# falgon/jpezy

Measured on AMD Instinct MI355X. Metric: Mpixels/s encode (FDCT+quant), higher is better.
Workload: dtype f32+f64 guard; 1 GPU; BASELINE configs[1]: single 4096x4096 random-pixel frame encode; width=4096, height=4096, mode=color, ring_batches=6, inputs=iid uniform u8 r,g,b planes resident in HBM, parallelism=frames x1, submission=one launch per step, the K steps captured once and replayed as a hipGraph

## Files before the change

jpezy_amd/csrc/jpezy_entropy.hip:

```cpp
#include <hip/hip_runtime.h>
#include <stdint.h>

#include "jpezy_entropy.h"
#include "../../include/jpezy_constants.h"

namespace jpezy_dev {
namespace entropy {

struct alignas(16) LdsTables {
    uint32_t dc[2][16];
    uint32_t ac[2][256];
    uint32_t fast[2][1024];
};
static_assert(sizeof(LdsTables) <= sizeof(CodeTables) && sizeof(LdsTables) % 16 == 0, "table images must match");

__device__ __forceinline__ void load_tables(LdsTables& L, const CodeTables* T)
{
    const uint4* src = reinterpret_cast<const uint4*>(T);
    uint4* dst = reinterpret_cast<uint4*>(&L);
    for (unsigned i = threadIdx.x; i < sizeof(LdsTables) / 16; i += blockDim.x) dst[i] = src[i];
}

__device__ __forceinline__ uint32_t wg256_exclusive_scan(uint32_t v, uint32_t* total)
{
    __shared__ uint32_t wsum[4];
    const int lane = threadIdx.x & 63, wv = threadIdx.x >> 6;
    uint32_t inc = v;
#pragma unroll
    for (int d = 1; d < 64; d <<= 1) {
        const uint32_t o = __shfl_up(inc, d, 64);
        if (lane >= d) inc += o;
    }
    if (lane == 63) wsum[wv] = inc;
    __syncthreads();
    uint32_t woff = 0, tot = 0;
#pragma unroll
    for (int k = 0; k < 4; ++k) {
        if (k < wv) woff += wsum[k];
        tot += wsum[k];
    }
    *total = tot;
    return woff + inc - v;
}

template <class W>
__device__ __forceinline__ void code_ac(uint32_t m, int base, const int16_t* z, int& prev, const uint32_t* ac, const uint32_t* fast,
                                        uint32_t zrl, W& w, unsigned& amax)
{
    int lz = __builtin_clz(m | 1u);
    int vnext = z[base + lz];
#pragma unroll 1
    while (m) {
        const int n = base + lz, v = vnext;
        m &= 0x7FFFFFFFu >> lz;
        lz = __builtin_clz(m | 1u);
        vnext = z[base + lz];
        w.read_up_to(n);
        int run = n - prev - 1;
        prev = n;
        const unsigned v32 = (unsigned)(v + 32);
        uint32_t e = fast[((unsigned)run << 6) + v32];
        const bool slow = v32 > 63u || run > 15;
        if (slow) {
            const unsigned a = (unsigned)(v < 0 ? -v : v);
            amax = a > amax ? a : amax;
            int sz = 32 - __builtin_clz(a);
            sz = sz > 10 ? 10 : sz;
            if (run > 15) {
                for (int r = run >> 4; r > 0; --r) w.put(zrl >> 8, (int)(zrl & 0xFF));
                run &= 15;
            }
            const uint32_t g = ac[(run << 4) | sz];
            e = ((((g >> 8) << sz) | ((uint32_t)(v + (v >> 31)) & ((1u << sz) - 1u))) << 5) | ((g & 0xFF) + (uint32_t)sz);
        }
        w.put(e >> 5, (int)(e & 31u));
    }
}

template <class W>
__device__ __forceinline__ bool code_block(const int16_t* z, int pred, const uint32_t* dc, const uint32_t* ac, const uint32_t* fast, W& w)
{
    unsigned amax = 0;
    bool ok = true;
    uint32_t mhi = 0, mlo = 0;
    int dcv = 0;
    if (z) {
#pragma unroll
        for (int k = 0; k < 8; ++k) {
            const uint4 c = reinterpret_cast<const uint4*>(z)[k];
            const uint32_t wd[4] = { c.x, c.y, c.z, c.w };
            uint32_t m8 = 0;
#pragma unroll
            for (int j = 0; j < 4; ++j) {
                m8 |= ((wd[j] & 0xFFFFu) ? 1u : 0u) << (7 - 2 * j);
                m8 |= ((wd[j] >> 16) ? 1u : 0u) << (6 - 2 * j);
            }
            if (k < 4) mhi |= m8 << (24 - 8 * k); else mlo |= m8 << (24 - 8 * (k - 4));
            if (k == 0) dcv = (int)(short)(c.x & 0xFFFFu);
        }
        mhi &= 0x7FFFFFFFu;
    }
    {
        const int diff = dcv - pred;
        const unsigned a = (unsigned)(diff < 0 ? -diff : diff);
        int di = a ? 32 - __builtin_clz(a) : 0;
        ok = di <= 11;
        di = di > 11 ? 11 : di;
        const uint32_t e = dc[di];
        w.put(((e >> 8) << di) | ((uint32_t)(diff + (diff >> 31)) & ((1u << di) - 1u)), (int)(e & 0xFF) + di);
    }
    int prev = 0;
    if (z) {
        const uint32_t zrl = ac[0xF0];
        code_ac(mhi, 0, z, prev, ac, fast, zrl, w, amax);
        code_ac(mlo, 32, z, prev, ac, fast, zrl, w, amax);
    }
    w.read_up_to(63);
    if (prev != 63) {
        const uint32_t e = ac[0x00];
        w.put(e >> 8, (int)(e & 0xFF));
    }
    return ok && amax <= 1023u;
}

constexpr int CHUNK = 64;

__device__ __forceinline__ unsigned count_ff(uint32_t x)
{
    const uint32_t z = ~x;
    uint32_t y = (z & 0x7F7F7F7Fu) + 0x7F7F7F7Fu;
    y = ~(y | z | 0x7F7F7F7Fu);
    return (unsigned)__builtin_popcount(y);
}

constexpr int WG = 256;
constexpr int ROW = 144, ROW_DATA = 16, ROW_LAST_WORD = 34;
constexpr unsigned TILE_STREAM_WORDS = 256 * kMaxBlockBytes / 4;

struct RowWriter {
    unsigned long long acc;
    int nacc, wj2, npos;
    unsigned long long bad;
    char* row12;
    __device__ __forceinline__ void init(uint32_t* r)
    {
        row12 = reinterpret_cast<char*>(r) + 12; acc = 0; nacc = 0; bad = 0;
        wj2 = -6; npos = 0;
    }
    __device__ __forceinline__ void read_up_to(int n) { npos = n; }
    __device__ __forceinline__ void word(uint32_t v, bool due)
    {
        const unsigned long long dm = __builtin_amdgcn_ballot_w64(due), lm = __builtin_amdgcn_ballot_w64(wj2 <= npos);
        if (due && wj2 <= npos) *reinterpret_cast<uint32_t*>(row12 + 2 * wj2) = v;
        bad |= dm & ~lm;
        wj2 += due ? 2 : 0;
    }
    __device__ __forceinline__ void put(uint32_t bits, int n)
    {
        acc = (acc << n) | bits;
        const int t = nacc + n;
        nacc = t & 31;
        word((uint32_t)(acc >> nacc), t >= 32);
    }
    __device__ __forceinline__ unsigned bits() const { return 16u * (unsigned)(wj2 + 6) + (unsigned)nacc; }
    __device__ __forceinline__ void finish()
    {
        word((uint32_t)(acc << (32 - nacc)), nacc > 0);
    }
    __device__ __forceinline__ bool overflowed() const { return (bad >> (threadIdx.x & 63u)) & 1ull; }
};

struct DirectWriter {
    unsigned long long acc;
    int nacc;
    unsigned w;
    uint32_t* S;
    bool skip;
    __device__ __forceinline__ void init(uint32_t* tile_stream, unsigned bitoff)
    {
        S = tile_stream; w = bitoff >> 5; nacc = (int)(bitoff & 31u); acc = 0; skip = nacc != 0;
    }
    __device__ __forceinline__ void read_up_to(int) {}
    __device__ __forceinline__ void put(uint32_t bits, int n)
    {
        acc = (acc << n) | bits;
        nacc += n;
        if (nacc >= 32) {
            nacc -= 32;
            if (!skip) S[w] = (uint32_t)(acc >> nacc);
            skip = false;
            ++w;
        }
    }
};

template <bool RST, unsigned CODED = 6u, unsigned LUMA = 4u>
__global__ __launch_bounds__(WG) void code_tiles_kernel(Job job, uint32_t* S, uint32_t* tile_total, unsigned* status)
{
    __shared__ LdsTables L;
    __shared__ __attribute__((aligned(16))) char tile[WG * ROW];
    const unsigned tid = threadIdx.x, frame = blockIdx.y;
    load_tables(L, job.tables + (size_t)frame * job.tables_stride);
    const unsigned nblk = job.blocks_per_frame;
    unsigned g0, nb;
    bool interval_start = false;
    if constexpr (RST) {
        const unsigned bpi = job.restart * CODED, tpi = restart_tpi<CODED>(job.restart), iv = blockIdx.x / tpi, j = blockIdx.x - iv * tpi;
        const unsigned i0 = iv * bpi, ilen = nblk - i0 < bpi ? nblk - i0 : bpi;
        g0 = i0 + j * (unsigned)WG;
        nb = ilen - j * (unsigned)WG < (unsigned)WG ? ilen - j * (unsigned)WG : (unsigned)WG;
        interval_start = j == 0;
    } else {
        g0 = blockIdx.x * (unsigned)WG;
        nb = nblk - g0 < (unsigned)WG ? nblk - g0 : (unsigned)WG;
    }
    const int16_t* fc = job.coeffs + (size_t)frame * job.coeffs_per_frame;
    const bool valid = tid < nb;
    int pred = 0, table = 0;
    const int16_t* zg = nullptr;
    if (valid) {
        const unsigned g = g0 + tid, mcu = g / CODED, i = g - mcu * CODED;
        table = i < LUMA ? 0 : 1;
        if (!(CODED == 6u && i >= 4 && job.bpm == 4)) {
            zg = fc + ((size_t)mcu * job.bpm + i) * 64;
            if (i >= 1 && i < LUMA) pred = zg[-64];
            else if (RST ? !(interval_start && tid < CODED) : mcu != 0) pred = i == 0 ? zg[-(job.bpm - (int)(LUMA - 1u)) * 64] : zg[-job.bpm * 64];
        }
    }
    if (CODED != 6u || job.bpm == 6) {
        const uint4* src = reinterpret_cast<const uint4*>(fc + (size_t)g0 * 64);
        for (unsigned c = tid; c < nb * 8u; c += WG)
            *reinterpret_cast<uint4*>(tile + (c >> 3) * ROW + ROW_DATA + (c & 7u) * 16u) = src[c];
    } else {
        const unsigned g1 = g0 + nb - 1, m0 = g0 / 6u, i0 = g0 - m0 * 6u, m1 = g1 / 6u, i1 = g1 - m1 * 6u;
        const unsigned s0 = i0 < 4 ? m0 * 4u + i0 : (m0 + 1) * 4u, s1 = i1 < 4 ? m1 * 4u + i1 : m1 * 4u + 3u;
        const unsigned nchunks = (s1 + 1 - s0) * 8u;
        const uint4* src = reinterpret_cast<const uint4*>(fc + (size_t)s0 * 64);
        for (unsigned c = tid; c < nchunks; c += WG) {
            const unsigned sb = s0 + (c >> 3), r = (sb >> 2) * 6u + (sb & 3u) - g0;
            *reinterpret_cast<uint4*>(tile + r * ROW + ROW_DATA + (c & 7u) * 16u) = src[c];
        }
    }
    __syncthreads();

    uint32_t* const row = reinterpret_cast<uint32_t*>(tile + tid * ROW);
    unsigned n = 0;
    bool ovf = false;
    if (valid) {
        RowWriter w;
        w.init(row);
        const bool ok = code_block(zg ? reinterpret_cast<const int16_t*>(tile + tid * ROW + ROW_DATA) : nullptr, pred, L.dc[table], L.ac[table],
                                   L.fast[table], w);
        n = w.bits();
        w.finish();
        ovf = w.overflowed();
        if (!ok) atomicOr(status + frame, 1u);
    }
    row[ROW_LAST_WORD + 1] = n;
    uint32_t total;
    const uint32_t o = wg256_exclusive_scan(n, &total);
    const size_t t_index = (size_t)frame * gridDim.x + blockIdx.x;
    if (tid == 0) tile_total[t_index] = total;
    if (!valid) return;

    uint32_t* const Sg = RST ? S + (size_t)frame * ((size_t)((nblk + 255u) / 256u) * TILE_STREAM_WORDS) + (size_t)g0 * (TILE_STREAM_WORDS / 256u)
                             : S + t_index * TILE_STREAM_WORDS;
    const unsigned sh = o & 31u, w0 = o >> 5, end = o + n;
    uint32_t tail = 0;
    unsigned tail_word = 0, tail_fill = 0;
    if (!ovf) {
        const unsigned nwp = (n + 31u) >> 5;
        unsigned k = sh ? 1u : 0u;
        uint32_t prev = sh ? row[0] : 0u;
        for (; ((w0 + k + 1u) << 5) <= end; ++k) {
            const uint32_t cur = k < nwp ? row[k] : 0u;
            Sg[w0 + k] = __builtin_amdgcn_alignbit(prev, cur, sh);
            prev = cur;
        }
        if (((w0 + k) << 5) < end) {
            const uint32_t cur = k < nwp ? row[k] : 0u;
            tail_word = w0 + k;
            tail_fill = end - (tail_word << 5);
            tail = __builtin_amdgcn_alignbit(prev, cur, sh) & ~(0xFFFFFFFFu >> tail_fill);
        }
    } else {
        DirectWriter w;
        w.init(Sg, o);
        (void)code_block(zg, pred, L.dc[table], L.ac[table], L.fast[table], w);
        if (w.nacc > 0 && !w.skip) {
            tail_word = w.w;
            tail_fill = (unsigned)w.nacc;
            tail = (uint32_t)(w.acc << (32 - w.nacc));
        }
    }
    if (tail_fill) {
        unsigned fill = tail_fill;
        for (unsigned j = tid + 1; fill < 32u && j < nb; ++j) {
            const uint32_t* rj = reinterpret_cast<const uint32_t*>(tile + j * ROW);
            tail |= rj[0] >> fill;
            fill += rj[ROW_LAST_WORD + 1];
        }
        Sg[tail_word] = tail;
    }
}

constexpr unsigned ASM_BITS = 256u * (unsigned)CHUNK * 8u;
__global__ __launch_bounds__(256) void tile_bases_kernel(const uint32_t* tile_total, unsigned tpf, unsigned long long* base,
                                                        unsigned long long* bytes, uint32_t* first_tile, unsigned ft_stride,
                                                        unsigned* status, unsigned* latched)
{
    const unsigned f = blockIdx.x, tid = threadIdx.x;
    const uint32_t* tt = tile_total + (size_t)f * tpf;
    unsigned long long* B = base + (size_t)f * (tpf + 1);
    uint32_t* ft = first_tile + (size_t)f * ft_stride;
    unsigned long long carry = 0;
    for (unsigned b0 = 0; b0 < tpf; b0 += 2048u) {
        uint32_t v[8], s = 0;
#pragma unroll
        for (int k = 0; k < 8; ++k) {
            const unsigned t = b0 + tid * 8u + k;
            v[k] = t < tpf ? tt[t] : 0u;
            s += v[k];
        }
        uint32_t total;
        unsigned long long run = carry + wg256_exclusive_scan(s, &total);
#pragma unroll
        for (int k = 0; k < 8; ++k) {
            const unsigned t = b0 + tid * 8u + k;
            if (t < tpf) {
                B[t] = run;
                for (unsigned long long w = (run + ASM_BITS - 1) / ASM_BITS; w * ASM_BITS < run + v[k] && w < ft_stride; ++w) ft[w] = t;
            }
            run += v[k];
        }
        carry += total;
        __syncthreads();
    }
    if (tid == 0) {
        B[tpf] = carry;
        bytes[f] = (carry + 7) >> 3;
        if (latched) {
            latched[f] = status[f];
            status[f] = 0;
        }
    }
}

constexpr unsigned MIN_TILE_BITS = 42u * 32u + 20u;
constexpr int ASM_WIN = 128;
static_assert((unsigned)(ASM_WIN - 2) * MIN_TILE_BITS >= ASM_BITS, "assemble window too small for flat content");
constexpr unsigned MIN_TILE_BITS_444 = 85u * 14u + 4u;
static_assert((unsigned)(ASM_WIN - 2) * MIN_TILE_BITS_444 >= ASM_BITS, "assemble window too small for flat 4:4:4 content");
constexpr unsigned MIN_TILE_BITS_ANY = 256u * 2u;
constexpr int ASM_WIN_ANY = 264;
static_assert((unsigned)(ASM_WIN_ANY - 2) * MIN_TILE_BITS_ANY >= ASM_BITS, "assemble window too small for one-bit codes");
constexpr unsigned ASM_SELF_TILES = 2048;

__device__ __forceinline__ unsigned assemble_chunk(unsigned long long p, unsigned long long bA, unsigned long long eA, const uint32_t* srcA,
                                                   unsigned LB, const uint32_t* srcB, unsigned long long T, uint4* dst)
{
    const unsigned long long qA = p - bA;
    const unsigned LA = (unsigned)(eA - bA), aA = (unsigned)(qA >> 5), sA = (unsigned)(qA & 31u);
    uint32_t wa[17];
#pragma unroll
    for (int k = 0; k < 17; ++k) wa[k] = qA < LA && ((aA + k) << 5) < LA ? srcA[aA + k] : 0u;
    const bool two = LB != 0 && p + CHUNK * 8 > eA;
    const unsigned dB = two ? (unsigned)(eA - p) : 0u, kb = dB >> 5, rb = dB & 31u;
    uint32_t wn[16];
#pragma unroll
    for (int k = 0; k < 16; ++k) wn[k] = two && (unsigned)k >= kb && (((unsigned)k - kb) << 5) < LB ? srcB[(unsigned)k - kb] : 0u;
    uint32_t out[16];
#pragma unroll
    for (int k = 0; k < 16; ++k) {
        uint32_t v = sA ? __builtin_amdgcn_alignbit(wa[k], wa[k + 1], 32u - sA) : wa[k];
        v |= __builtin_amdgcn_alignbit(k > 0 ? wn[k - 1] : 0u, wn[k], rb);
        out[k] = v;
    }
#if JPEZY_PAD_BIT
    {
        const unsigned pad = (unsigned)((8 - (T & 7)) & 7);
        if (pad && T > p && T < p + CHUNK * 8) {
            const unsigned kk = (unsigned)((T - p) >> 5), keep = (unsigned)((T - p) & 31u);
#pragma unroll
            for (int k = 0; k < 16; ++k)
                if ((unsigned)k == kk) out[k] |= ((1u << pad) - 1u) << (32u - keep - pad);
        }
    }
#else
    (void)T;
#endif
    unsigned n_ff = 0;
#pragma unroll
    for (int k = 0; k < 16; ++k) n_ff += count_ff(out[k]);
#pragma unroll
    for (int k = 0; k < 4; ++k)
        dst[k] = make_uint4(__builtin_bswap32(out[4 * k]), __builtin_bswap32(out[4 * k + 1]), __builtin_bswap32(out[4 * k + 2]),
                            __builtin_bswap32(out[4 * k + 3]));
    return n_ff;
}

template <bool SELF, int WIN = ASM_WIN>
__global__ __launch_bounds__(256) void assemble_kernel(const uint32_t* S, const uint32_t* tile_total, const unsigned long long* base,
                                                      unsigned long long* bytes, const uint32_t* first_tile, unsigned tpf,
                                                      unsigned ft_stride, uint32_t* U, size_t u_stride_words, uint32_t* loc,
                                                      uint32_t* ff_tile_total, unsigned* status, unsigned* latched)
{
    __shared__ unsigned long long wb[SELF ? 1 : WIN + 2];
    __shared__ uint32_t pre[SELF ? ASM_SELF_TILES + 2 : 1];
    const unsigned frame = blockIdx.y, tid = threadIdx.x;
    const size_t chunks_per_frame = u_stride_words * 4 / CHUNK, pieces = chunks_per_frame / 256;
    unsigned long long T, nbytes;
    if constexpr (SELF) {
        const uint32_t* tt = tile_total + (size_t)frame * tpf;
        uint32_t v[8], sum = 0;
#pragma unroll
        for (int k = 0; k < 8; ++k) {
            const unsigned t = tid * 8u + k;
            v[k] = t < tpf ? tt[t] : 0u;
            sum += v[k];
        }
        uint32_t total;
        uint32_t run = wg256_exclusive_scan(sum, &total);
#pragma unroll
        for (int k = 0; k < 8; ++k) {
            pre[tid * 8u + k] = run;
            run += v[k];
        }
        if (tid == 255) { pre[ASM_SELF_TILES] = total; pre[ASM_SELF_TILES + 1] = total; }
        __syncthreads();
        T = total;
        nbytes = (T + 7) >> 3;
        if (blockIdx.x == 0 && tid == 0) {
            bytes[frame] = nbytes;
            if (latched) {
                latched[frame] = status[frame];
                status[frame] = 0;
            }
        }
    } else {
        nbytes = bytes[frame];
        T = 0;
#if JPEZY_PAD_BIT
        T = base[(size_t)frame * (tpf + 1) + tpf];
#endif
    }
    for (size_t x = blockIdx.x; x < pieces; x += gridDim.x) {
        const unsigned long long c0 = (unsigned long long)x * 256u, c = c0 + tid;
        if (x != 0 && c0 * CHUNK > nbytes) break;
        unsigned n_ff = 0;
        const unsigned long long p = c * (CHUNK * 8ull);
        uint4* dst = reinterpret_cast<uint4*>(U + (size_t)frame * u_stride_words) + c * (CHUNK / 16);
        if constexpr (SELF) {
            if (c * CHUNK < nbytes) {
                unsigned lo = 0, hi = tpf;
                while (hi - lo > 1) {
                    const unsigned mid = (lo + hi) >> 1;
                    if (pre[mid] <= p) lo = mid; else hi = mid;
                }
                const unsigned t = lo;
                const uint32_t* srcA = S + ((size_t)frame * tpf + t) * TILE_STREAM_WORDS;
                const unsigned LB = t + 1 < tpf ? pre[t + 2] - pre[t + 1] : 0u;
                n_ff = assemble_chunk(p, pre[t], pre[t + 1], srcA, LB, srcA + TILE_STREAM_WORDS, T, dst);
            }
        } else {
            const unsigned t0 = first_tile[(size_t)frame * ft_stride + x];
            const unsigned long long* B = base + (size_t)frame * (tpf + 1);
            __syncthreads();
            for (unsigned i = tid; i < (unsigned)WIN + 2u; i += 256u) wb[i] = B[t0 + i < tpf ? t0 + i : tpf];
            __syncthreads();
            if (c * CHUNK < nbytes) {
                int lo = 0, hi = WIN;
                while (hi - lo > 1) {
                    const int mid = (lo + hi) >> 1;
                    if (wb[mid] <= p) lo = mid; else hi = mid;
                }
                const int t = lo;
                const unsigned tA = t0 + (unsigned)t < tpf ? t0 + (unsigned)t : tpf - 1;
                const uint32_t* srcA = S + ((size_t)frame * tpf + tA) * TILE_STREAM_WORDS;
                const unsigned LB = tA + 1 < tpf ? (unsigned)(wb[t + 2] - wb[t + 1]) : 0u;
                n_ff = assemble_chunk(p, wb[t], wb[t + 1], srcA, LB, srcA + TILE_STREAM_WORDS, T, dst);
            }
        }
        uint32_t total;
        const uint32_t off = wg256_exclusive_scan(n_ff, &total);
        loc[(size_t)frame * chunks_per_frame + c] = off;
        if (tid == 0) ff_tile_total[(size_t)frame * pieces + x] = total;
        __syncthreads();
    }
}

__global__ __launch_bounds__(256) void restart_bases_kernel(const uint32_t* tile_total, unsigned tpf, unsigned tpi, unsigned ni,
                                                           unsigned long long* base, unsigned long long* padsum, unsigned long long* bytes,
                                                           uint32_t* first_tile, unsigned ft_stride, unsigned* status, unsigned* latched)
{
    const unsigned f = blockIdx.x, tid = threadIdx.x;
    const uint32_t* tt = tile_total + (size_t)f * tpf;
    unsigned long long* B = base + (size_t)f * (tpf + 1);
    unsigned long long* P = padsum + (size_t)f * ni;
    uint32_t* ft = first_tile + (size_t)f * ft_stride;
    unsigned long long carry = 0;
    for (unsigned b0 = 0; b0 < tpf; b0 += 2048u) {
        uint32_t v[8], s = 0;
#pragma unroll
        for (int k = 0; k < 8; ++k) {
            const unsigned t = b0 + tid * 8u + k;
            v[k] = t < tpf ? tt[t] : 0u;
            s += v[k];
        }
        uint32_t total;
        unsigned long long run = carry + wg256_exclusive_scan(s, &total);
#pragma unroll
        for (int k = 0; k < 8; ++k) {
            const unsigned t = b0 + tid * 8u + k;
            if (t < tpf) B[t] = run;
            run += v[k];
        }
        carry += total;
        __syncthreads();
    }
    if (tid == 0) B[tpf] = carry;
    __syncthreads();
    carry = 0;
    for (unsigned k0 = 0; k0 < ni; k0 += 2048u) {
        uint32_t v[8], s = 0;
#pragma unroll
        for (int e = 0; e < 8; ++e) {
            const unsigned k = k0 + tid * 8u + e;
            v[e] = k + 1 < ni ? (uint32_t)((0ull - (B[(size_t)(k + 1) * tpi] - B[(size_t)k * tpi])) & 7ull) : 0u;
            s += v[e];
        }
        uint32_t total;
        unsigned long long run = carry + wg256_exclusive_scan(s, &total);
#pragma unroll
        for (int e = 0; e < 8; ++e) {
            const unsigned k = k0 + tid * 8u + e;
            if (k < ni) P[k] = run;
            run += v[e];
        }
        carry += total;
        __syncthreads();
    }
    for (unsigned t = tid; t <= tpf; t += 256u) {
        const unsigned k = t / tpi;
        B[t] += P[k < ni ? k : ni - 1];
    }
    __syncthreads();
    for (unsigned t = tid; t < tpf; t += 256u) {
        const unsigned long long b = B[t], e = B[t + 1];
        for (unsigned long long w = (b + ASM_BITS - 1) / ASM_BITS; w * ASM_BITS < e && w < ft_stride; ++w) ft[w] = t;
    }
    if (tid == 0) {
        bytes[f] = (B[tpf] + 7) >> 3;
        if (latched) {
            latched[f] = status[f];
            status[f] = 0;
        }
    }
}

template <unsigned CODED>
__device__ __forceinline__ unsigned assemble_chunk_restart(unsigned long long p, const unsigned long long* B, const uint32_t* tt, unsigned t,
                                                           unsigned tpf, unsigned tpi, unsigned restart, const uint32_t* Sf,
                                                           unsigned long long T, uint4* dst, unsigned long long& marks, unsigned& k7)
{
    uint32_t out[16];
#pragma unroll
    for (int k = 0; k < 16; ++k) out[k] = 0u;
    marks = 0;
    k7 = 0;
    unsigned long long b = B[t];
    for (unsigned u = t; u < tpf && b < p + CHUNK * 8; ++u) {
        const unsigned long long e = B[u + 1];
        const uint32_t* src = Sf + (size_t)restart_tile_first<CODED>(u, restart) * (TILE_STREAM_WORDS / 256u);
        const unsigned L = tt[u];
        if (u == t) {
            const unsigned long long q = p - b;
            const unsigned a = (unsigned)(q >> 5), sa = (unsigned)(q & 31u);
            uint32_t wa[17];
#pragma unroll
            for (int k = 0; k < 17; ++k) wa[k] = ((a + k) << 5) < L ? src[a + k] : 0u;
#pragma unroll
            for (int k = 0; k < 16; ++k) out[k] = sa ? __builtin_amdgcn_alignbit(wa[k], wa[k + 1], 32u - sa) : wa[k];
        } else {
            const unsigned d = (unsigned)(b - p), kb = d >> 5, rb = d & 31u;
            uint32_t wn[16];
#pragma unroll
            for (int k = 0; k < 16; ++k) wn[k] = (unsigned)k >= kb && (((unsigned)k - kb) << 5) < L ? src[(unsigned)k - kb] : 0u;
#pragma unroll
            for (int k = 0; k < 16; ++k) out[k] |= __builtin_amdgcn_alignbit(k > 0 ? wn[k - 1] : 0u, wn[k], rb);
        }
        const bool ends = (u + 1) % tpi == 0 && u + 1 < tpf;
        if (ends && e <= p + CHUNK * 8) {
            if (!marks) k7 = (u / tpi) & 7u;
            marks |= 1ull << (unsigned)(((e - p) >> 3) - 1);
        }
#if JPEZY_PAD_BIT
        if (ends) {
            const unsigned long long raw = b + L;
            const unsigned pad = (unsigned)(e - raw);
            if (pad && raw < p + CHUNK * 8) {
                const unsigned kk = (unsigned)((raw - p) >> 5), keep = (unsigned)((raw - p) & 31u);
#pragma unroll
                for (int k = 0; k < 16; ++k)
                    if ((unsigned)k == kk) out[k] |= ((1u << pad) - 1u) << (32u - keep - pad);
            }
        }
#endif
        b = e;
    }
#if JPEZY_PAD_BIT
    {
        const unsigned pad = (unsigned)((8 - (T & 7)) & 7);
        if (pad && T > p && T < p + CHUNK * 8) {
            const unsigned kk = (unsigned)((T - p) >> 5), keep = (unsigned)((T - p) & 31u);
#pragma unroll
            for (int k = 0; k < 16; ++k)
                if ((unsigned)k == kk) out[k] |= ((1u << pad) - 1u) << (32u - keep - pad);
        }
    }
#else
    (void)T;
#endif
    unsigned n_ff = 0;
#pragma unroll
    for (int k = 0; k < 16; ++k) n_ff += count_ff(out[k]);
#pragma unroll
    for (int k = 0; k < 4; ++k)
        dst[k] = make_uint4(__builtin_bswap32(out[4 * k]), __builtin_bswap32(out[4 * k + 1]), __builtin_bswap32(out[4 * k + 2]),
                            __builtin_bswap32(out[4 * k + 3]));
    return n_ff + 2u * (unsigned)__builtin_popcountll(marks);
}

template <unsigned CODED>
__global__ __launch_bounds__(256) void assemble_restart_kernel(const uint32_t* S, size_t s_frame_words, const uint32_t* tile_total,
                                                              const unsigned long long* base, const unsigned long long* bytes,
                                                              const uint32_t* first_tile, unsigned tpf, unsigned restart, unsigned ft_stride,
                                                              uint32_t* U, size_t u_stride_words, uint32_t* loc, uint32_t* ff_tile_total,
                                                              unsigned long long* markers)
{
    const unsigned frame = blockIdx.y, tid = threadIdx.x;
    const size_t chunks_per_frame = u_stride_words * 4 / CHUNK, pieces = chunks_per_frame / 256;
    const unsigned long long* B = base + (size_t)frame * (tpf + 1);
    const uint32_t* ft = first_tile + (size_t)frame * ft_stride;
    const unsigned long long nbytes = bytes[frame], T = B[tpf];
    const unsigned tpi = restart_tpi<CODED>(restart);
    for (size_t x = blockIdx.x; x < pieces; x += gridDim.x) {
        const unsigned long long c0 = (unsigned long long)x * 256u, c = c0 + tid;
        if (x != 0 && c0 * CHUNK > nbytes) break;
        unsigned extra = 0, k7 = 0;
        unsigned long long marks = 0;
        const unsigned long long p = c * (CHUNK * 8ull);
        if (c * CHUNK < nbytes) {
            unsigned lo = ft[x], hi = (unsigned long long)(x + 1) * ASM_BITS < T ? ft[x + 1] + 1u : tpf;
            while (hi - lo > 1) {
                const unsigned mid = (lo + hi) >> 1;
                if (B[mid] <= p) lo = mid; else hi = mid;
            }
            uint4* dst = reinterpret_cast<uint4*>(U + (size_t)frame * u_stride_words) + c * (CHUNK / 16);
            extra = assemble_chunk_restart<CODED>(p, B, tile_total + (size_t)frame * tpf, lo, tpf, tpi, restart, S + (size_t)frame * s_frame_words, T,
                                           dst, marks, k7);
        }
        uint32_t total;
        const uint32_t off = wg256_exclusive_scan(extra, &total);
        loc[(size_t)frame * chunks_per_frame + c] = off | (k7 << 29);
        markers[(size_t)frame * chunks_per_frame + c] = marks;
        if (tid == 0) ff_tile_total[(size_t)frame * pieces + x] = total;
        __syncthreads();
    }
}

constexpr int SCAN_T = 256, SCAN_E = 8, SCAN_N = SCAN_T * SCAN_E;

template <typename TIn>
__global__ __launch_bounds__(SCAN_T) void scan_local_kernel(const TIn* in, unsigned long long* out, unsigned long long* totals,
                                                           size_t n)
{
    __shared__ unsigned long long wsum[SCAN_T / 64];
    const size_t base = (size_t)blockIdx.x * SCAN_N + (size_t)threadIdx.x * SCAN_E;
    unsigned long long v[SCAN_E], s = 0;
#pragma unroll
    for (int k = 0; k < SCAN_E; ++k) {
        v[k] = base + k < n ? (unsigned long long)in[base + k] : 0ull;
        s += v[k];
    }
    unsigned long long inc = s;
    const int lane = threadIdx.x & 63, wv = threadIdx.x >> 6;
#pragma unroll
    for (int d = 1; d < 64; d <<= 1) {
        const unsigned long long o = __shfl_up(inc, d, 64);
        if (lane >= d) inc += o;
    }
    if (lane == 63) wsum[wv] = inc;
    __syncthreads();
    unsigned long long woff = 0;
    for (int k = 0; k < wv; ++k) woff += wsum[k];
    unsigned long long run = woff + inc - s;
#pragma unroll
    for (int k = 0; k < SCAN_E; ++k) {
        if (base + k < n) out[base + k] = run;
        run += v[k];
    }
    if (threadIdx.x == SCAN_T - 1) {
        totals[blockIdx.x] = run;
        if (gridDim.x == 1) out[n] = run;
    }
}

__global__ __launch_bounds__(SCAN_T) void scan_add_kernel(unsigned long long* out, const unsigned long long* offs, size_t n,
                                                         unsigned long long* total_slot)
{
    const size_t base = (size_t)blockIdx.x * SCAN_N + (size_t)threadIdx.x * SCAN_E;
    const unsigned long long o = offs[blockIdx.x];
#pragma unroll
    for (int k = 0; k < SCAN_E; ++k)
        if (base + k < n) out[base + k] += o;
    (void)total_slot;
}

size_t scan_tmp_elems(size_t n)
{
    size_t t = 0;
    while (n > 1) {
        n = (n + SCAN_N - 1) / SCAN_N;
        t += n + 1 + n;
        if (n == 1) break;
    }
    return t + 4;
}

__global__ __launch_bounds__(SCAN_T) void scan_finish_kernel(unsigned long long* out, const unsigned long long* totals, size_t n, size_t nb)
{
    __shared__ unsigned long long wsum[SCAN_T / 64];
    unsigned long long sum = 0;
    for (size_t k = threadIdx.x; k < (size_t)blockIdx.x; k += SCAN_T) sum += totals[k];
#pragma unroll
    for (int d = 32; d >= 1; d >>= 1) sum += __shfl_xor(sum, d, 64);
    if ((threadIdx.x & 63) == 0) wsum[threadIdx.x >> 6] = sum;
    __syncthreads();
    unsigned long long o = 0;
#pragma unroll
    for (int k = 0; k < SCAN_T / 64; ++k) o += wsum[k];
    const size_t base = (size_t)blockIdx.x * SCAN_N + (size_t)threadIdx.x * SCAN_E;
#pragma unroll
    for (int k = 0; k < SCAN_E; ++k)
        if (base + k < n) out[base + k] += o;
    if (blockIdx.x == nb - 1 && threadIdx.x == 0) out[n] = o + totals[nb - 1];
}

constexpr size_t SCAN_ONE_WG_MAX = 16 * SCAN_N;
template <typename TIn>
__global__ __launch_bounds__(SCAN_T) void scan_one_wg_kernel(const TIn* in, unsigned long long* out, size_t n)
{
    __shared__ unsigned long long wsum[SCAN_T / 64];
    const int lane = threadIdx.x & 63, wv = threadIdx.x >> 6;
    unsigned long long carry = 0;
    for (size_t b0 = 0; b0 < n; b0 += SCAN_N) {
        const size_t base = b0 + (size_t)threadIdx.x * SCAN_E;
        unsigned long long v[SCAN_E], s = 0;
#pragma unroll
        for (int k = 0; k < SCAN_E; ++k) {
            v[k] = base + k < n ? (unsigned long long)in[base + k] : 0ull;
            s += v[k];
        }
        unsigned long long inc = s;
#pragma unroll
        for (int d = 1; d < 64; d <<= 1) {
            const unsigned long long o = __shfl_up(inc, d, 64);
            if (lane >= d) inc += o;
        }
        if (lane == 63) wsum[wv] = inc;
        __syncthreads();
        unsigned long long woff = 0, tot = 0;
#pragma unroll
        for (int k = 0; k < SCAN_T / 64; ++k) {
            if (k < wv) woff += wsum[k];
            tot += wsum[k];
        }
        unsigned long long run = carry + woff + inc - s;
#pragma unroll
        for (int k = 0; k < SCAN_E; ++k) {
            if (base + k < n) out[base + k] = run;
            run += v[k];
        }
        carry += tot;
        __syncthreads();
    }
    if (threadIdx.x == 0) out[n] = carry;
}

constexpr size_t SCAN_FINISH_MAX_WGS = 4096;

template <typename TIn>
static hipError_t scan_exclusive(const TIn* in, unsigned long long* out, size_t n, unsigned long long* tmp, hipStream_t s)
{
    if (n == 0) return hipMemsetAsync(out, 0, sizeof(unsigned long long), s);
    if (n <= SCAN_ONE_WG_MAX) {
        hipLaunchKernelGGL((scan_one_wg_kernel<TIn>), dim3(1), dim3(SCAN_T), 0, s, in, out, n);
        return hipGetLastError();
    }
    const size_t nb = (n + SCAN_N - 1) / SCAN_N;
    unsigned long long* raw = tmp;
    unsigned long long* scanned = tmp + nb;
    hipLaunchKernelGGL((scan_local_kernel<TIn>), dim3((unsigned)nb), dim3(SCAN_T), 0, s, in, out, raw, n);
    if (nb == 1) return hipGetLastError();
    if (nb <= SCAN_FINISH_MAX_WGS) {
        hipLaunchKernelGGL(scan_finish_kernel, dim3((unsigned)nb), dim3(SCAN_T), 0, s, out, raw, n, nb);
        return hipGetLastError();
    }
    hipError_t e = scan_exclusive<unsigned long long>(raw, scanned, nb, scanned + nb + 1, s);
    if (e != hipSuccess) return e;
    hipLaunchKernelGGL(scan_add_kernel, dim3((unsigned)nb), dim3(SCAN_T), 0, s, out, scanned, n, (unsigned long long*)nullptr);
    return hipMemcpyAsync(out + n, scanned + nb, sizeof(unsigned long long), hipMemcpyDeviceToDevice, s);
}


constexpr int STUFF_WG = 256;
template <bool RST>
__global__ __launch_bounds__(STUFF_WG) void stuff_kernel(const uint32_t* U, size_t u_stride_words, const unsigned long long* frame_bytes,
                                                        const uint32_t* ff_loc, const uint32_t* ff_tile_total, uint8_t* out, size_t out_stride,
                                                        FilePlan plan)
{
    __shared__ uint32_t buf[STUFF_WG * CHUNK * (RST ? 3 : 2) / 4 + 4];
    __shared__ unsigned long long red[2][STUFF_WG / 64];
    uint8_t* const lb = reinterpret_cast<uint8_t*>(buf);
    const size_t chunks_per_frame = u_stride_words * 4 / CHUNK, pieces = chunks_per_frame / STUFF_WG;
    const size_t frame = blockIdx.y;
    const unsigned long long nbytes = frame_bytes[frame];
    for (size_t px = blockIdx.x; (unsigned long long)px * STUFF_WG * CHUNK < nbytes; px += gridDim.x) {
        const size_t c0 = px * STUFF_WG, c = c0 + threadIdx.x;
        const uint32_t* loc = ff_loc + frame * chunks_per_frame;
        const bool has_data = (unsigned long long)c * CHUNK < nbytes;
        uint4 data[CHUNK / 16];
        uint32_t my_loc = 0;
        unsigned long long marks = 0;
        unsigned k7 = 0;
        if (has_data) {
            const uint4* src = reinterpret_cast<const uint4*>(reinterpret_cast<const uint8_t*>(U + frame * u_stride_words) + c * CHUNK);
#pragma unroll
            for (int k = 0; k < CHUNK / 16; ++k) data[k] = src[k];
            my_loc = loc[c];
            if constexpr (RST) {
                marks = plan.markers[frame * chunks_per_frame + c];
                k7 = my_loc >> 29;
                my_loc &= 0x1FFFFFFFu;
            }
        }
        const uint32_t* ft = ff_tile_total + frame * pieces;
        const size_t last = (size_t)(nbytes / ((unsigned long long)STUFF_WG * CHUNK)), used = last + 1 < pieces ? last + 1 : pieces;
        unsigned long long pre = 0, all = 0;
        for (size_t x = threadIdx.x; x < used; x += STUFF_WG) {
            const uint32_t v = ft[x];
            all += v;
            pre += x < px ? v : 0u;
        }
#pragma unroll
        for (int d = 32; d >= 1; d >>= 1) {
            pre += __shfl_xor(pre, d, 64);
            all += __shfl_xor(all, d, 64);
        }
        if ((threadIdx.x & 63) == 0) { red[0][threadIdx.x >> 6] = pre; red[1][threadIdx.x >> 6] = all; }
        __syncthreads();
        pre = all = 0;
#pragma unroll
        for (int k = 0; k < STUFF_WG / 64; ++k) { pre += red[0][k]; all += red[1][k]; }
        if (plan.hdr) {
            const unsigned long long body = nbytes + all;
            const unsigned long long total = plan.hdr_len + body + 2;
            const unsigned st = plan.latched[frame];
            const bool failed = st != 0 || total > out_stride;
            if (px == 0) {
                uint8_t* file = out + frame * out_stride;
                if (threadIdx.x == 0) {
                    plan.sizes[frame] = st ? -5 : failed ? -6 : (long long)total;
                    if (!failed) {
                        file[plan.hdr_len + body] = 0xFF;
                        file[plan.hdr_len + body + 1] = 0xD9;
                    }
                }
                if (!failed)
                    for (size_t i = threadIdx.x; i < plan.hdr_len; i += STUFF_WG) file[i] = plan.hdr[i];
            }
            if (failed) return;
        }
        uint8_t* const P = out + (plan.hdr ? plan.hdr_len : 0) + frame * out_stride + c0 * CHUNK + pre;
        const unsigned shift = (unsigned)(reinterpret_cast<uintptr_t>(P) & 3u);
        if (has_data) {
            const int n = (int)((nbytes - (unsigned long long)c * CHUNK) < (unsigned long long)CHUNK ? (nbytes - (unsigned long long)c * CHUNK) : CHUNK);
            uint8_t* dst = lb + shift + threadIdx.x * CHUNK + my_loc;
#pragma unroll
            for (int k = 0; k < CHUNK / 16; ++k) {
                const uint32_t wd[4] = { data[k].x, data[k].y, data[k].z, data[k].w };
#pragma unroll
                for (int j = 0; j < 16; ++j) {
                    if (k * 16 + j < n) {
                        const uint8_t b = (uint8_t)(wd[j >> 2] >> ((j & 3) * 8));
                        *dst++ = b;
                        if (b == 0xFF) *dst++ = 0x00;
                        if constexpr (RST) {
                            if ((marks >> (k * 16 + j)) & 1ull) {
                                *dst++ = 0xFF;
                                *dst++ = (uint8_t)(0xD0u + k7);
                                k7 = (k7 + 1u) & 7u;
                            }
                        }
                    }
                }
            }
        }
        __syncthreads();
        const unsigned long long last_chunk = (nbytes + CHUNK - 1) / CHUNK;
        const size_t ce = c0 + STUFF_WG < last_chunk ? c0 + STUFF_WG : (size_t)last_chunk;
        const unsigned long long src_end = (unsigned long long)ce * CHUNK < nbytes ? (unsigned long long)ce * CHUNK : nbytes;
        const unsigned total = (unsigned)(src_end - (unsigned long long)c0 * CHUNK) + (ce < c0 + STUFF_WG ? (RST ? loc[ce] & 0x1FFFFFFFu : loc[ce]) : ft[px]);
        uint32_t* const A = reinterpret_cast<uint32_t*>(P - shift);
        const unsigned end = shift + total, nwords = (end + 3) / 4;
        for (unsigned w = threadIdx.x; w < nwords; w += STUFF_WG) {
            const unsigned lo = w * 4, hi = lo + 4;
            if (lo >= shift && hi <= end) {
                A[w] = buf[w];
            } else {
                for (unsigned k = lo < shift ? shift : lo; k < (hi < end ? hi : end); ++k) reinterpret_cast<uint8_t*>(A)[k] = lb[k];
            }
        }
        __syncthreads();
    }
}

hipError_t launch_scan_u32(const uint32_t* in, unsigned long long* out, size_t n, unsigned long long* tmp, hipStream_t s)
{
    hipError_t e = scan_exclusive<uint32_t>(in, out, n, tmp, s);
    return e != hipSuccess ? e : hipGetLastError();
}

size_t chunk_bytes() { return CHUNK; }
size_t assemble_piece_bytes() { return (size_t)256 * CHUNK; }

static bool assemble_scans_tiles_itself(const Job& job) { return !job.restart && job_tiles(job) <= ASM_SELF_TILES; }

size_t stream_stride(const Job& job)
{
    const size_t worst = (size_t)job.blocks_per_frame * kMaxBlockBytes + (job.restart ? restart_intervals(job.blocks_per_frame, job.restart, (unsigned)job.coded) : 0);
    return (worst + 8 + assemble_piece_bytes() - 1) / assemble_piece_bytes() * assemble_piece_bytes();
}

size_t max_pass_frames(const Job& job)
{
    const size_t n = ((size_t)1 << 30) / stream_stride(job);
    return n ? n : 1;
}

ScratchSizes scratch_sizes(const Job& job, bool)
{
    const size_t F = (size_t)job.n_frames, u_stride = stream_stride(job), pieces = u_stride / assemble_piece_bytes(), chunks = u_stride / CHUNK;
    const bool self = assemble_scans_tiles_itself(job);
    ScratchSizes z;
    z.tile_stream = tiles256(job.blocks_per_frame) * F * TILE_STREAM_WORDS * sizeof(uint32_t);
    z.tile_total = job_tiles(job) * F * sizeof(uint32_t);
    z.tile_base = self ? 0 : (job_tiles(job) + 1) * F * sizeof(unsigned long long);
    z.first_tile = self ? 0 : pieces * F * sizeof(uint32_t);
    z.restart_pad = job.restart ? restart_intervals(job.blocks_per_frame, job.restart, (unsigned)job.coded) * F * sizeof(unsigned long long) : 0;
    z.bytes = F * sizeof(unsigned long long);
    z.U = u_stride * F;
    z.ff_loc = chunks * F * sizeof(uint32_t);
    z.ff_piece = pieces * F * sizeof(uint32_t);
    z.markers = job.restart ? chunks * F * sizeof(unsigned long long) : 0;
    z.flags = F * sizeof(unsigned);
    return z;
}

hipError_t launch_code_tiles(const Job& job, const Scratch& sc, hipStream_t s)
{
    if (!job.blocks_per_frame || job.n_frames <= 0) return hipSuccess;
    if (job.n_frames > 65535 || !layout_ok(job)) return hipErrorInvalidValue;
    const unsigned coded = (unsigned)job.coded;
    const dim3 grid((unsigned)job_tiles(job), (unsigned)job.n_frames);
    if (job.restart) {
        if (job.restart > 65535u || job.blocks_per_frame % coded || job.restart >= job.blocks_per_frame / coded) return hipErrorInvalidValue;
        if (coded == 3u) hipLaunchKernelGGL((code_tiles_kernel<true, 3u, 1u>), grid, dim3(WG), 0, s, job, sc.tile_stream, sc.tile_total, sc.status);
        else hipLaunchKernelGGL(code_tiles_kernel<true>, grid, dim3(WG), 0, s, job, sc.tile_stream, sc.tile_total, sc.status);
    } else if (coded == 3u)
        hipLaunchKernelGGL((code_tiles_kernel<false, 3u, 1u>), grid, dim3(WG), 0, s, job, sc.tile_stream, sc.tile_total, sc.status);
    else
        hipLaunchKernelGGL(code_tiles_kernel<false>, grid, dim3(WG), 0, s, job, sc.tile_stream, sc.tile_total, sc.status);
    return hipGetLastError();
}

hipError_t launch_tile_bases(const Job& job, const Scratch& sc, hipStream_t s)
{
    if (!job.blocks_per_frame || job.n_frames <= 0 || assemble_scans_tiles_itself(job)) return hipSuccess;
    if (job.restart) {
        if (!layout_ok(job) || job.restart >= job.blocks_per_frame / (unsigned)job.coded) return hipErrorInvalidValue;
        hipLaunchKernelGGL(restart_bases_kernel, dim3((unsigned)job.n_frames), dim3(256), 0, s, sc.tile_total, (unsigned)job_tiles(job),
                           restart_tpi_of(job.restart, (unsigned)job.coded),
                           (unsigned)restart_intervals(job.blocks_per_frame, job.restart, (unsigned)job.coded), sc.tile_base, sc.restart_pad,
                           sc.bytes, sc.first_tile, sc.ft_stride, sc.status, sc.latched);
    } else
        hipLaunchKernelGGL(tile_bases_kernel, dim3((unsigned)job.n_frames), dim3(256), 0, s, sc.tile_total, (unsigned)job_tiles(job), sc.tile_base,
                           sc.bytes, sc.first_tile, sc.ft_stride, sc.status, sc.latched);
    return hipGetLastError();
}

hipError_t launch_assemble(const Job& job, const Scratch& sc, bool any_tables, hipStream_t s)
{
    const size_t pieces = sc.u_stride / assemble_piece_bytes(), u_stride_words = sc.u_stride / 4;
    const unsigned tpf = (unsigned)job_tiles(job);
    if (!pieces || job.n_frames <= 0) return hipSuccess;
    if (sc.u_stride % assemble_piece_bytes() || job.n_frames > 65535) return hipErrorInvalidValue;
    size_t gx = pieces < 1024 ? pieces : 1024;
    if (job.n_frames > 1 && gx > 128) gx = 128;
    const dim3 grid((unsigned)gx, (unsigned)job.n_frames);
    if (assemble_scans_tiles_itself(job)) {
        hipLaunchKernelGGL(assemble_kernel<true>, grid, dim3(256), 0, s, sc.tile_stream, sc.tile_total, sc.tile_base, sc.bytes, sc.first_tile, tpf,
                           sc.ft_stride, sc.U, u_stride_words, sc.ff_loc, sc.ff_piece, sc.status, sc.latched);
        return hipGetLastError();
    }
    if (pieces > sc.ft_stride) return hipErrorInvalidValue;
    if (job.restart && job.coded == 3)
        hipLaunchKernelGGL(assemble_restart_kernel<3u>, grid, dim3(256), 0, s, sc.tile_stream, tiles256(job.blocks_per_frame) * (size_t)TILE_STREAM_WORDS,
                           sc.tile_total, sc.tile_base, sc.bytes, sc.first_tile, tpf, job.restart, sc.ft_stride, sc.U, u_stride_words, sc.ff_loc,
                           sc.ff_piece, sc.markers);
    else if (job.restart)
        hipLaunchKernelGGL(assemble_restart_kernel<6u>, grid, dim3(256), 0, s, sc.tile_stream, tiles256(job.blocks_per_frame) * (size_t)TILE_STREAM_WORDS,
                           sc.tile_total, sc.tile_base, sc.bytes, sc.first_tile, tpf, job.restart, sc.ft_stride, sc.U, u_stride_words, sc.ff_loc,
                           sc.ff_piece, sc.markers);
    else if (any_tables)
        hipLaunchKernelGGL((assemble_kernel<false, ASM_WIN_ANY>), grid, dim3(256), 0, s, sc.tile_stream, sc.tile_total, sc.tile_base, sc.bytes,
                           sc.first_tile, tpf, sc.ft_stride, sc.U, u_stride_words, sc.ff_loc, sc.ff_piece, sc.status, sc.latched);
    else
        hipLaunchKernelGGL(assemble_kernel<false>, grid, dim3(256), 0, s, sc.tile_stream, sc.tile_total, sc.tile_base, sc.bytes, sc.first_tile, tpf,
                           sc.ft_stride, sc.U, u_stride_words, sc.ff_loc, sc.ff_piece, sc.status, sc.latched);
    return hipGetLastError();
}

hipError_t launch_stuff(const Job& job, const Scratch& sc, uint8_t* out, size_t out_stride, FilePlan plan, hipStream_t s)
{
    const size_t chunks = sc.u_stride / CHUNK;
    if (!chunks || job.n_frames <= 0) return hipSuccess;
    if (job.n_frames > 65535 || chunks % STUFF_WG) return hipErrorInvalidValue;
    size_t gx = chunks / STUFF_WG < 1024 ? chunks / STUFF_WG : 1024;
    if (job.n_frames > 1 && gx > 128) gx = 128;
    plan.latched = sc.latched;
    plan.markers = job.restart ? sc.markers : nullptr;
    if (plan.markers)
        hipLaunchKernelGGL(stuff_kernel<true>, dim3((unsigned)gx, (unsigned)job.n_frames), dim3(STUFF_WG), 0, s, sc.U, sc.u_stride / 4, sc.bytes,
                           sc.ff_loc, sc.ff_piece, out, out_stride, plan);
    else
        hipLaunchKernelGGL(stuff_kernel<false>, dim3((unsigned)gx, (unsigned)job.n_frames), dim3(STUFF_WG), 0, s, sc.U, sc.u_stride / 4, sc.bytes,
                           sc.ff_loc, sc.ff_piece, out, out_stride, plan);
    return hipGetLastError();
}

__global__ __launch_bounds__(256) void ff_frame_totals_kernel(const uint32_t* ff_tile_total, const unsigned long long* bytes, size_t pieces,
                                                             unsigned long long* dst)
{
    __shared__ unsigned long long red[4];
    const size_t piece_bytes = (size_t)256 * CHUNK;
    const size_t used = (size_t)(bytes[blockIdx.x] / piece_bytes) + 1 < pieces ? (size_t)(bytes[blockIdx.x] / piece_bytes) + 1 : pieces;
    unsigned long long sum = 0;
    for (size_t x = threadIdx.x; x < used; x += 256) sum += ff_tile_total[blockIdx.x * pieces + x];
#pragma unroll
    for (int d = 32; d >= 1; d >>= 1) sum += __shfl_xor(sum, d, 64);
    if ((threadIdx.x & 63) == 0) red[threadIdx.x >> 6] = sum;
    __syncthreads();
    if (threadIdx.x == 0) dst[blockIdx.x] = red[0] + red[1] + red[2] + red[3];
}

hipError_t launch_ff_frame_totals(const Job& job, const Scratch& sc, unsigned long long* dst, hipStream_t s)
{
    if (job.n_frames <= 0) return hipSuccess;
    hipLaunchKernelGGL(ff_frame_totals_kernel, dim3((unsigned)job.n_frames), dim3(256), 0, s, sc.ff_piece, sc.bytes,
                       sc.u_stride / assemble_piece_bytes(), dst);
    return hipGetLastError();
}

}
}
```

Measured before the change: 643,700 Mpixels/s.

## Split each assemble chunk across four lanes for coalesced loads and stores

```diff
diff --git a/jpezy_amd/csrc/jpezy_entropy.hip b/jpezy_amd/csrc/jpezy_entropy.hip
--- a/jpezy_amd/csrc/jpezy_entropy.hip
+++ b/jpezy_amd/csrc/jpezy_entropy.hip
@@ -356,25 +356,28 @@
 static_assert((unsigned)(ASM_WIN_ANY - 2) * MIN_TILE_BITS_ANY >= ASM_BITS, "assemble window too small for one-bit codes");
 constexpr unsigned ASM_SELF_TILES = 2048;
 
-__device__ __forceinline__ unsigned assemble_chunk(unsigned long long p, unsigned long long bA, unsigned long long eA, const uint32_t* srcA,
-                                                   unsigned LB, const uint32_t* srcB, unsigned long long T, uint4* dst)
+__device__ __forceinline__ unsigned assemble_quarter(unsigned long long p, unsigned long long bA, unsigned long long eA, const uint32_t* srcA,
+                                                     unsigned LB, const uint32_t* srcB, unsigned long long T, unsigned q, uint4* dst)
 {
     const unsigned long long qA = p - bA;
-    const unsigned LA = (unsigned)(eA - bA), aA = (unsigned)(qA >> 5), sA = (unsigned)(qA & 31u);
-    uint32_t wa[17];
-#pragma unroll
-    for (int k = 0; k < 17; ++k) wa[k] = qA < LA && ((aA + k) << 5) < LA ? srcA[aA + k] : 0u;
+    const unsigned LA = (unsigned)(eA - bA), aA = (unsigned)(qA >> 5) + 4u * q, sA = (unsigned)(qA & 31u);
+    uint32_t wa[5];
+#pragma unroll
+    for (int k = 0; k < 5; ++k) wa[k] = qA < LA && ((aA + k) << 5) < LA ? srcA[aA + k] : 0u;
     const bool two = LB != 0 && p + CHUNK * 8 > eA;
     const unsigned dB = two ? (unsigned)(eA - p) : 0u, kb = dB >> 5, rb = dB & 31u;
-    uint32_t wn[16];
-#pragma unroll
-    for (int k = 0; k < 16; ++k) wn[k] = two && (unsigned)k >= kb && (((unsigned)k - kb) << 5) < LB ? srcB[(unsigned)k - kb] : 0u;
-    uint32_t out[16];
-#pragma unroll
-    for (int k = 0; k < 16; ++k) {
-        uint32_t v = sA ? __builtin_amdgcn_alignbit(wa[k], wa[k + 1], 32u - sA) : wa[k];
-        v |= __builtin_amdgcn_alignbit(k > 0 ? wn[k - 1] : 0u, wn[k], rb);
-        out[k] = v;
+    uint32_t wn[5];
+#pragma unroll
+    for (int j = 0; j < 5; ++j) {
+        const int k = 4 * (int)q - 1 + j;
+        wn[j] = two && k >= (int)kb && (((unsigned)k - kb) << 5) < LB ? srcB[(unsigned)k - kb] : 0u;
+    }
+    uint32_t out[4];
+#pragma unroll
+    for (int j = 0; j < 4; ++j) {
+        uint32_t v = sA ? __builtin_amdgcn_alignbit(wa[j], wa[j + 1], 32u - sA) : wa[j];
+        v |= __builtin_amdgcn_alignbit(wn[j], wn[j + 1], rb);
+        out[j] = v;
     }
 #if JPEZY_PAD_BIT
     {
@@ -382,21 +385,15 @@
         if (pad && T > p && T < p + CHUNK * 8) {
             const unsigned kk = (unsigned)((T - p) >> 5), keep = (unsigned)((T - p) & 31u);
 #pragma unroll
-            for (int k = 0; k < 16; ++k)
-                if ((unsigned)k == kk) out[k] |= ((1u << pad) - 1u) << (32u - keep - pad);
+            for (int j = 0; j < 4; ++j)
+                if (4u * q + (unsigned)j == kk) out[j] |= ((1u << pad) - 1u) << (32u - keep - pad);
         }
     }
 #else
     (void)T;
 #endif
-    unsigned n_ff = 0;
-#pragma unroll
-    for (int k = 0; k < 16; ++k) n_ff += count_ff(out[k]);
-#pragma unroll
-    for (int k = 0; k < 4; ++k)
-        dst[k] = make_uint4(__builtin_bswap32(out[4 * k]), __builtin_bswap32(out[4 * k + 1]), __builtin_bswap32(out[4 * k + 2]),
-                            __builtin_bswap32(out[4 * k + 3]));
-    return n_ff;
+    *dst = make_uint4(__builtin_bswap32(out[0]), __builtin_bswap32(out[1]), __builtin_bswap32(out[2]), __builtin_bswap32(out[3]));
+    return count_ff(out[0]) + count_ff(out[1]) + count_ff(out[2]) + count_ff(out[3]);
 }
 
 template <bool SELF, int WIN = ASM_WIN>
@@ -407,6 +404,7 @@
 {
     __shared__ unsigned long long wb[SELF ? 1 : WIN + 2];
     __shared__ uint32_t pre[SELF ? ASM_SELF_TILES + 2 : 1];
+    __shared__ uint32_t tile_of[256], ff_of[256];
     const unsigned frame = blockIdx.y, tid = threadIdx.x;
     const size_t chunks_per_frame = u_stride_words * 4 / CHUNK, pieces = chunks_per_frame / 256;
     unsigned long long T, nbytes;
@@ -447,42 +445,52 @@
     for (size_t x = blockIdx.x; x < pieces; x += gridDim.x) {
         const unsigned long long c0 = (unsigned long long)x * 256u, c = c0 + tid;
         if (x != 0 && c0 * CHUNK > nbytes) break;
-        unsigned n_ff = 0;
         const unsigned long long p = c * (CHUNK * 8ull);
-        uint4* dst = reinterpret_cast<uint4*>(U + (size_t)frame * u_stride_words) + c * (CHUNK / 16);
-        if constexpr (SELF) {
-            if (c * CHUNK < nbytes) {
-                unsigned lo = 0, hi = tpf;
-                while (hi - lo > 1) {
-                    const unsigned mid = (lo + hi) >> 1;
-                    if (pre[mid] <= p) lo = mid; else hi = mid;
-                }
-                const unsigned t = lo;
-                const uint32_t* srcA = S + ((size_t)frame * tpf + t) * TILE_STREAM_WORDS;
-                const unsigned LB = t + 1 < tpf ? pre[t + 2] - pre[t + 1] : 0u;
-                n_ff = assemble_chunk(p, pre[t], pre[t + 1], srcA, LB, srcA + TILE_STREAM_WORDS, T, dst);
-            }
-        } else {
-            const unsigned t0 = first_tile[(size_t)frame * ft_stride + x];
+        unsigned t0 = 0;
+        if constexpr (!SELF) {
+            t0 = first_tile[(size_t)frame * ft_stride + x];
             const unsigned long long* B = base + (size_t)frame * (tpf + 1);
             __syncthreads();
             for (unsigned i = tid; i < (unsigned)WIN + 2u; i += 256u) wb[i] = B[t0 + i < tpf ? t0 + i : tpf];
             __syncthreads();
-            if (c * CHUNK < nbytes) {
-                int lo = 0, hi = WIN;
-                while (hi - lo > 1) {
-                    const int mid = (lo + hi) >> 1;
-                    if (wb[mid] <= p) lo = mid; else hi = mid;
+        }
+        if (c * CHUNK < nbytes) {
+            unsigned lo = 0, hi = SELF ? tpf : (unsigned)WIN;
+            while (hi - lo > 1) {
+                const unsigned mid = (lo + hi) >> 1;
+                bool le;
+                if constexpr (SELF) le = pre[mid] <= p; else le = wb[mid] <= p;
+                if (le) lo = mid; else hi = mid;
+            }
+            tile_of[tid] = lo;
+        }
+        __syncthreads();
+        uint4* const dst = reinterpret_cast<uint4*>(U + (size_t)frame * u_stride_words) + c0 * (CHUNK / 16);
+#pragma unroll
+        for (unsigned j = 0; j < 4; ++j) {
+            const unsigned ch = j * 64u + (tid >> 2), q = tid & 3u;
+            const unsigned long long cq = c0 + ch, pq = cq * (CHUNK * 8ull);
+            unsigned n = 0;
+            if (cq * CHUNK < nbytes) {
+                const unsigned t = tile_of[ch];
+                if constexpr (SELF) {
+                    const uint32_t* srcA = S + ((size_t)frame * tpf + t) * TILE_STREAM_WORDS;
+                    const unsigned LB = t + 1 < tpf ? pre[t + 2] - pre[t + 1] : 0u;
+                    n = assemble_quarter(pq, pre[t], pre[t + 1], srcA, LB, srcA + TILE_STREAM_WORDS, T, q, dst + ch * (CHUNK / 16) + q);
+                } else {
+                    const unsigned tA = t0 + t < tpf ? t0 + t : tpf - 1;
+                    const uint32_t* srcA = S + ((size_t)frame * tpf + tA) * TILE_STREAM_WORDS;
+                    const unsigned LB = tA + 1 < tpf ? (unsigned)(wb[t + 2] - wb[t + 1]) : 0u;
+                    n = assemble_quarter(pq, wb[t], wb[t + 1], srcA, LB, srcA + TILE_STREAM_WORDS, T, q, dst + ch * (CHUNK / 16) + q);
                 }
-                const int t = lo;
-                const unsigned tA = t0 + (unsigned)t < tpf ? t0 + (unsigned)t : tpf - 1;
-                const uint32_t* srcA = S + ((size_t)frame * tpf + tA) * TILE_STREAM_WORDS;
-                const unsigned LB = tA + 1 < tpf ? (unsigned)(wb[t + 2] - wb[t + 1]) : 0u;
-                n_ff = assemble_chunk(p, wb[t], wb[t + 1], srcA, LB, srcA + TILE_STREAM_WORDS, T, dst);
-            }
-        }
+            }
+            n += __shfl_xor(n, 1, 64);
+            n += __shfl_xor(n, 2, 64);
+            if (q == 0) ff_of[ch] = n;
+        }
+        __syncthreads();
         uint32_t total;
-        const uint32_t off = wg256_exclusive_scan(n_ff, &total);
+        const uint32_t off = wg256_exclusive_scan(ff_of[tid], &total);
         loc[(size_t)frame * chunks_per_frame + c] = off;
         if (tid == 0) ff_tile_total[(size_t)frame * pieces + x] = total;
         __syncthreads();
```

New measurement: 644,100 Mpixels/s, median of 2. Within noise of the previous version (+0.1%).
